# MeshFEM/MeshFEM

Measured on AMD Instinct MI355X. Metric: stiffness_assembly_elements_per_s, higher is better.
Workload: dtype f64; 1 GPU; configs[2]: 60^3 grid -> 5184000 P2 tets, isotropic E=200 nu=0.35, Dirichlet x=0, traction x=1; elements=5184000, nodes=7430761, dof=22292283, nnz_blocks=201443041, stored_blocks=104436901, matrix_storage=upper, parallelism=1 GPU, step=embed + Ke blocks + assembly into block-CSR (gather/owner-computes)

## Files before the change

### meshfem_amd/csrc/mfh_api.cpp

```cpp
#include "mfh_ctx.hh"
#include <dlfcn.h>

using namespace mfh;

namespace {
struct RoctxApi {
    int (*push)(const char *) = nullptr;
    int (*pop)() = nullptr;
    RoctxApi() {
        const char *en = getenv("MFH_ROCTX");
        if (!en || en[0] == '0') return;
        for (const char *lib : {"librocprofiler-sdk-roctx.so", "libroctx64.so", "/opt/rocm/lib/librocprofiler-sdk-roctx.so", "/opt/rocm/lib/libroctx64.so"}) {
            if (void *h = dlopen(lib, RTLD_NOW | RTLD_GLOBAL)) {
                push = reinterpret_cast<int (*)(const char *)>(dlsym(h, "roctxRangePushA"));
                pop = reinterpret_cast<int (*)()>(dlsym(h, "roctxRangePop"));
                if (push && pop) return;
                push = nullptr; pop = nullptr;
            }
        }
    }
};
RoctxApi &roctx_api() { static RoctxApi a; return a; }
}
mfh::RoctxRange::RoctxRange(const char *name) {
// ... 68 lines not shown
    double t0 = now_ms();
    c->autoStretch = -1.0;
    drop_p1_view(c);
    c->opDegree = 0;
    c->nodePairsValid = false;
    sampler_drop(c);
    if (!c->hostOnly && !deviceTables) {
        require_device(c);
        MFH_HIP(hipSetDevice(c->device));
        c->dElemNodes.upload(c->mesh.elemNodes, c->stream);
        c->dVertPos.upload(c->mesh.nodePos, c->stream);
    }
    c->timing.upload_ms = now_ms() - t0;
    c->haveMesh = true;
    c->external = false;
    c->geoValid = false;
    c->hGeoValid = false;
    c->dofForNode.clear();
    c->nDoF = c->mesh.nNode;
    build_shape_tables(c->mesh.dim, c->mesh.deg, c->tables);
    if (!c->hostOnly) { c->dPairTable.upload(c->tables.pairTable, c->stream); c->dMassTable.upload(c->tables.massRef, c->stream); }
    invalidate_symbolic(c);
    dist_detach(c);
    reset_bcs(c);
    clear_fixed(c);
}

void set_isotropic(mfh_ctx *c, double E, double nu) {
    double lam = (nu * E) / ((1.0 + nu) * (1.0 - 2.0 * nu));
    if (c->haveMesh && c->mesh.dim == 2) lam = (nu * E) / (1.0 - nu * nu);
    c->matMode = 0;
    c->matKind = MAT_ISO;
    c->matParams = {lam, E / (2.0 + 2.0 * nu), E, nu};
    c->geoValid = false;
    c->hGeoValid = false;
    invalidate_matrix(c);
}

void drop_p1_view(mfh_ctx *c) {
    if (c->p1) { mfh_destroy(c->p1); c->p1 = nullptr; }
    c->p1GeoGen = -1;
}

mfh_ctx *p1_view(mfh_ctx *c) {
    if (!c || c->opDegree != 1 || !c->p1) return nullptr;
    mfh_ctx *v = c->p1;
    if (!c->hostOnly) {
        ensure_geometry(c);
        v->dGeo.borrow(c->dGeo.p, c->dGeo.n);
        v->geoStride = c->geoStride;
        v->geoValid = true;
        if (v->dVertPos.borrowed || !v->dVertPos.p) v->dVertPos.borrow(c->dVertPos.p, (size_t)v->mesh.nNode * v->mesh.dim);
        if (c->p1GeoGen != c->geoGen) { invalidate_matrix(v); c->p1GeoGen = c->geoGen; }
    }
    return v;
}

void ensure_pass_events(mfh_ctx *c) {
    if (c->passEv[0]) return;
    for (auto &e : c->passEv) MFH_HIP(hipEventCreate(&e));
    MFH_HIP(hipHostMalloc((void **)&c->negHost, 2 * sizeof(int), hipHostMallocDefault));
}

void ensure_geometry(mfh_ctx *c, bool deferCheck) {
    require(c->haveMesh, MFH_ERR_STATE, "no mesh set");
    if (c->geoValid) return;
    require(!c->hostOnly, MFH_ERR_HIP, "host-only context (device -1): no HIP device, and there is no CPU fallback");
    require_device(c);
    MFH_HIP(hipSetDevice(c->device));
    const HostMesh &m = c->mesh;
    if (c->matParams.empty() && !c->dMatBorrowed) set_isotropic(c, 1.0, 0.3);
    if (c->matMode == 0 && !c->dMatBorrowed) {
        double E = c->matParams[2], nu = c->matParams[3];
        double lam = (nu * E) / ((1.0 + nu) * (1.0 - 2.0 * nu));
        if (m.dim == 2) lam = (nu * E) / (1.0 - nu * nu);
        c->matParams[0] = lam;
    }
    c->geoStride = c->matKind == MAT_ISO ? GEO_ISO_STRIDE : (c->matKind == MAT_ORTHO ? GEO_ORTHO_STRIDE : GEO_GEN_STRIDE);
    if (!c->dMatBorrowed) c->dMatParams.upload(c->matParams, c->stream);
    const double *dMat = c->dMatBorrowed ? c->dMatBorrowed : c->dMatParams.p;
    c->dGeo.alloc((size_t)m.nElem * c->geoStride);
    c->dNeg.alloc(2);
    c->dNeg.zero(c->stream);
    ensure_pass_events(c);
    MFH_HIP(hipEventRecord(c->passEv[0], c->stream));
    k::launch_geometry(m.dim, m.deg, c->matKind, m.nElem, c->dElemNodes.p, m.npe, c->dVertPos.p, dMat, c->matMode,
                       c->dGeo.p, c->geoStride, c->dNeg.p, c->stream);
    MFH_HIP(hipEventRecord(c->passEv[1], c->stream));
    MFH_HIP(hipMemcpyAsync(c->negHost, c->dNeg.p, 2 * sizeof(int), hipMemcpyDeviceToHost, c->stream));
    c->geoPending = true;
    if (!deferCheck) finish_geometry(c);
}

void finish_geometry(mfh_ctx *c) {
    if (!c->geoPending) return;
    c->geoPending = false;
    MFH_HIP(hipStreamSynchronize(c->stream));
    float ms = 0;
    MFH_HIP(hipEventElapsedTime(&ms, c->passEv[0], c->passEv[1]));
    c->timing.geometry_ms = ms;
    const int neg[2] = {c->negHost[0], c->negHost[1]};
    if (neg[0] > 0)
        throw Error(MFH_ERR_INVALID, "Mesh has negatively oriented elements.\nCorrect with: mesh_convert --reorientNegativeElements. (" +
                                         std::to_string(neg[0]) + " elements)");
    if (neg[1] > 0)
        throw Error(MFH_ERR_INVALID, std::string(c->matMode == 1 ? "Isotropic" : "Orthotropic") + " parameters of " + std::to_string(neg[1]) +
                                         " elements give an indefinite elasticity tensor (" +
                                         (c->matMode == 1 ? "need E > 0 and -1 < nu < 1/2, nu < 1 in plane stress" : "compliance matrix not positive definite") + ").");
    c->geoValid = true;
    c->hGeoValid = false;
    ++c->geoGen;
}

const std::vector<double> &host_geo(mfh_ctx *c) {
    ensure_geometry(c);
    if (!c->hGeoValid) {
        c->hGeo.resize(c->dGeo.n);
        c->dGeo.download(c->hGeo.data(), c->dGeo.n, c->stream);
        c->hGeoValid = true;
    }
    return c->hGeo;
}

const int32_t *device_dof_map(mfh_ctx *c) {
    if (c->dofForNode.empty()) return nullptr;
    if (!c->dofUploaded) { c->dDofForNode.upload(c->dofForNode, c->stream); c->dofUploaded = true; }
    return c->dDofForNode.p;
}

void ensure_host_colidx(mfh_ctx *c) {
    if (!c->sym.colIdx.empty() || c->sym.nnzb == 0) return;
    c->sym.colIdx.resize((size_t)c->sym.nnzb);
    c->dColIdx.download(c->sym.colIdx.data(), c->sym.colIdx.size(), c->stream);
}
// ... 78 lines not shown
    flag.alloc(1);
    c->codesPacked = k::launch_pack_codes(c->sym.nChunk(), c->dContribPtr.p, c->dContribCode.p, c->mesh.npe, c->dChunkElemBase.p, flag.p, c->stream);
}

void ensure_node_pairs(mfh_ctx *c) {
    if (c->nodePairsValid) return;
    const HostMesh &m = c->mesh;
    const int npe = m.npe;
    std::vector<int32_t> ptr((size_t)m.nNode + 1, 0), pairs((size_t)m.nElem * npe);
    require((int64_t)pairs.size() <= 2147483647LL, MFH_ERR_UNSUPPORTED, "more than 2^31 (element, node) pairs");
    for (size_t k2 = 0; k2 < pairs.size(); ++k2) ++ptr[(size_t)m.elemNodes[k2] + 1];
    for (int64_t n = 0; n < m.nNode; ++n) ptr[(size_t)n + 1] += ptr[(size_t)n];
    std::vector<int32_t> cur(ptr.begin(), ptr.end() - 1);
    for (size_t k2 = 0; k2 < pairs.size(); ++k2) pairs[(size_t)cur[(size_t)m.elemNodes[k2]]++] = (int32_t)k2;
    c->dNodePtr.upload(ptr, c->stream);
    c->dNodePair.upload(pairs, c->stream);
    c->nodePairsValid = true;
}

k::AsmArgs asm_args(mfh_ctx *c) {
    const HostMesh &m = c->mesh;
    k::AsmArgs a{};
    a.dim = m.dim; a.deg = m.deg; a.npe = m.npe; a.mat = c->asmMat();
    a.geoStride = c->geoStride; a.geo = c->dGeo.p; a.pairTable = c->dPairTable.p; a.massTable = c->dMassTable.p;
    for (int k2 = 0; k2 < 6; ++k2) a.pairConst[k2] = c->tables.pairConst[k2];
    a.nChunk = c->sym.nChunk(); a.chunkRow = c->dChunkRow.p; a.rowPtr = c->dRowPtr.p;
    a.contribPtr = c->dContribPtr.p; a.contribCode = c->dContribCode.p; a.contribSlot = c->dContribSlot.p;
    a.chunkSlots = c->sym.chunkSlots;
    a.nElem = m.nElem; a.scatterSlot = c->dScatter.p;
    a.vals = c->dVals.p; a.nnzb = c->sym.nnzb;
    a.xcd = c->xcdSwizzle;
    a.upperOnly = c->upperOnly ? 1 : 0;
    a.det = c->deterministic ? 1 : 0;
    a.chunkElemBase = c->codesPacked ? c->dChunkElemBase.p : nullptr;
    a.chunkOrder = nullptr;
    if (c->asmChunkOrder && !c->hostOnly && a.nChunk > 1 && c->symValid && c->dContribPtr.p && c->dContribCode.p && c->contribOrder == 1) {
        if (c->chunkOrderGen != c->listsGen) {
            DBuf<uint32_t> keys;
            keys.alloc((size_t)a.nChunk);
            k::launch_chunk_keys(a, keys.p, c->stream);
            std::vector<uint32_t> hk((size_t)a.nChunk);
            keys.download(hk.data(), hk.size(), c->stream);
            std::vector<int32_t> order((size_t)a.nChunk);
            for (int64_t b = 0; b < a.nChunk; ++b) order[(size_t)b] = (int32_t)b;
            std::stable_sort(order.begin(), order.end(), [&](int32_t x, int32_t y) { return hk[(size_t)x] < hk[(size_t)y]; });
            c->dChunkOrder.upload(order, c->stream);
            c->chunkOrderGen = c->listsGen;
        }
        a.chunkOrder = c->dChunkOrder.p;
    }
    return a;
}

void run_assembly(mfh_ctx *c, int mode) {
    c->dVals32.release();
    k::AsmArgs a = asm_args(c);
    if (mode == MFH_ASSEMBLE_ATOMIC) {
        c->dVals.zero(c->stream);
        k::launch_assemble_atomic(a, c->stream);
    } else {
        k::launch_assemble_gather(a, c->stream);
    }
}

void placement_trials(mfh_ctx *c) {
    c->placementGen = c->valsGen;
// ... 866 lines not shown
    MFH_TRY(c)
    require(c && out, MFH_ERR_INVALID, "null argument");
    const std::vector<double> &g = host_geo(c);
    for (int64_t e = 0; e < c->mesh.nElem; ++e) out[e] = g[(size_t)e * c->geoStride + 12];
    MFH_CATCH(c)
}

mfh_status mfh_material_isotropic(mfh_ctx *c, double E, double nu) {
    MFH_TRY(c)
    require(c, MFH_ERR_INVALID, "null context");
    set_isotropic(c, E, nu);
    MFH_CATCH(c)
}

mfh_status mfh_material_const(mfh_ctx *c, const double *D) {
    MFH_TRY(c)
    require(c && D && c->haveMesh, MFH_ERR_STATE, "set the mesh before the material");
    const int d = c->dim(), fl = flat_len(d);
    c->matParams.clear();
    bool ortho = true;
    for (int r = 0; r < fl && ortho; ++r)
        for (int cc = r + 1; cc < fl; ++cc)
            if (cc >= d && D[r * fl + cc] != 0.0) { ortho = false; break; }
    if (ortho) {
        for (int r = 0; r < d; ++r)
            for (int cc = r; cc < d; ++cc) c->matParams.push_back(D[r * fl + cc]);
        for (int k2 = d; k2 < fl; ++k2) c->matParams.push_back(D[k2 * fl + k2]);
        c->matMode = 5; c->matKind = MAT_ORTHO;
    } else {
        for (int r = 0; r < fl; ++r)
            for (int cc = r; cc < fl; ++cc) c->matParams.push_back(D[r * fl + cc]);
        c->matMode = 2; c->matKind = MAT_GENERAL;
    }
    c->geoValid = false; c->hGeoValid = false;
    invalidate_matrix(c);
    MFH_CATCH(c)
}

mfh_status mfh_material_iso_field(mfh_ctx *c, const double *E, const double *nu) {
    MFH_TRY(c)
    require(c && E && nu && c->haveMesh, MFH_ERR_STATE, "set the mesh before the material");
    const int64_t n = c->mesh.nElem;
    c->matParams.assign((size_t)2 * n, 0.0);
    std::copy(E, E + n, c->matParams.begin());
    std::copy(nu, nu + n, c->matParams.begin() + n);
    c->matMode = 1; c->matKind = MAT_ISO;
    c->geoValid = false; c->hGeoValid = false;
    invalidate_matrix(c);
    MFH_CATCH(c)
}

mfh_status mfh_material_ortho_field(mfh_ctx *c, const double *params) {
    MFH_TRY(c)
    require(c && params && c->haveMesh, MFH_ERR_STATE, "set the mesh before the material");
    const int np = c->dim() == 3 ? 9 : 4;
    c->matParams.assign(params, params + (size_t)np * c->mesh.nElem);
    c->matMode = 3; c->matKind = MAT_ORTHO;
    c->geoValid = false; c->hGeoValid = false;
    invalidate_matrix(c);
    MFH_CATCH(c)
}

mfh_status mfh_material_tensor_field(mfh_ctx *c, const double *D) {
    MFH_TRY(c)
    require(c && D && c->haveMesh, MFH_ERR_STATE, "set the mesh before the material");
    const int fl = flat_len(c->dim());
    c->matParams.assign(D, D + (size_t)fl * fl * c->mesh.nElem);
    c->matMode = 4; c->matKind = MAT_GENERAL;
    c->geoValid = false; c->hGeoValid = false;
    invalidate_matrix(c);
    MFH_CATCH(c)
}

mfh_status mfh_material_get(mfh_ctx *c, int64_t elem, double *D) {
    MFH_TRY(c)
    require(c && D && c->haveMesh && elem >= 0 && elem < c->mesh.nElem, MFH_ERR_INVALID, "bad element");
    const std::vector<double> &g = host_geo(c);
    elem_D(c, &g[(size_t)elem * c->geoStride], D);
    MFH_CATCH(c)
}

mfh_status mfh_dof_map(mfh_ctx *c, const int32_t *dofForNode, int64_t nDoF) {
    MFH_TRY(c)
    require(!(c && c->opDegree == 1 && c->p1), MFH_ERR_STATE, "a forced-degree-1 view is in force (mfh_set_operator_degree): it is defined for the identity DoF map");
    require(c && c->haveMesh, MFH_ERR_STATE, "no mesh set");
    c->nOwnedDoFSet = -1;
    if (!dofForNode) {
        c->dofForNode.clear();
        c->nDoF = c->mesh.nNode;
        std::fill(c->mesh.bdryInternal.begin(), c->mesh.bdryInternal.end(), (uint8_t)0);
    } else {
        require(c->mesh.nOwned == c->mesh.nNode, MFH_ERR_UNSUPPORTED, "a DoF map on a partitioned mesh says which DoFs are this rank's rows: mfh_dof_map_partitioned");
        require(nDoF > 0 && nDoF <= c->mesh.nNode, MFH_ERR_INVALID, "bad nDoF");
        for (int64_t n = 0; n < c->mesh.nNode; ++n)
            require(dofForNode[n] >= 0 && dofForNode[n] < nDoF, MFH_ERR_INVALID, "DoF index out of range");
        c->dofForNode.assign(dofForNode, dofForNode + c->mesh.nNode);
        c->nDoF = nDoF;
    }
    invalidate_symbolic(c);
    clear_fixed(c);
    MFH_CATCH(c)
}
// ... 921 lines not shown
```

### meshfem_amd/csrc/mfh_ctx.hh

```
#pragma once
#include "mfh_internal.hh"
#include <cmath>
#include <map>
#include <mutex>

using namespace mfh;

struct mfh_ctx {
    int device = 0;
    bool hostOnly = false;
    bool hierarchyLevel = false;
    bool keepHostSymbolic = false;
    int xcdSwizzle = 0;
    RawVec<double> hLoad, hX, hXBatch, hLoadBatch;
    bool alwaysReembed = false;
    bool deterministic = false;
    DBuf<double> detPartials;
    DBuf<unsigned> detCounter;
    bool periodicIgnoreMismatch = false;
    int periodicIgnoreDims = 0;
    hipStream_t stream = nullptr;
    bool ownStream = true;
    bool arenaCounted = false;
    std::string err;

    HostMesh mesh;
    bool haveMesh = false;
    bool external = false;
    DBuf<int32_t> dElemNodes;
    DBuf<double> dVertPos;

    int matMode = 0;
    int matKind = MAT_ISO;
    int op = MFH_OP_ELASTICITY;
    int opDegree = 0;
    mfh_ctx *p1 = nullptr;
    int64_t geoGen = 0, p1GeoGen = -1;
    DBuf<int32_t> dNodePtr, dNodePair;
    bool nodePairsValid = false;
    struct SamplerGrid {
        bool valid = false;
        int nc[3] = {1, 1, 1};
        double org[3] = {0, 0, 0}, hi[3] = {0, 0, 0}, cs[3] = {1, 1, 1};
        int64_t nItems = 0, nPairs = 0, maxPop = 0;
        double buildMs = 0, hostMs = 0;
        DBuf<int32_t> cellStart, items;
        void reset() { valid = false; nItems = nPairs = maxPop = 0; buildMs = hostMs = 0; cellStart.release(); items.release(); }
    };
    struct Sampler {
        SamplerGrid elem, bdry;
        double pad = 0;
        double bbMin[3] = {0, 0, 0}, bbMax[3] = {0, 0, 0};
        DBuf<int32_t> bdryVerts, bdryParent;
    } sampler;
    double samplerCellScale = 1.0;
    std::vector<double> matParams;
    DBuf<double> dMatParams;
    const double *dMatBorrowed = nullptr;
    DBuf<double> dGeo;
    DBuf<int> dNeg;
    int geoStride = GEO_ISO_STRIDE;
    bool geoValid = false;
    hipEvent_t passEv[4] = {nullptr, nullptr, nullptr, nullptr};
    int *negHost = nullptr;
    bool geoPending = false;
    std::vector<double> hGeo;
    bool hGeoValid = false;

    std::vector<int32_t> dofForNode;
    DBuf<int32_t> dDofForNode;
    bool dofUploaded = false;
    int64_t nDoF = 0;

    Symbolic sym;
    bool symValid = false;
    bool symHasScatter = false;
    DBuf<int32_t> dRowPtr, dColIdx, dChunkRow, dSpmvChunkRow, dScatter;
    DBuf<int64_t> dContribPtr;
    int matrixStorage = -1;
    bool upperOnly = false;
    int nCU = 256;
    DBuf<uint32_t> dContribCode;
    DBuf<uint16_t> dContribSlot;
    ShapeTables tables;
    DBuf<double> dPairTable, dMassTable;
    MfLists mf;
    bool mfValid = false;
    int matrixFree = -1;
    bool use_mf() const {
        if (external || !haveMesh || hostOnly || kron()) return false;
        return matrixFree == 1 || (matrixFree < 0 && op == MFH_OP_ELASTICITY);
    }
    DBuf<int32_t> dMfChunkRow;
// ... 328 lines not shown
```

### meshfem_amd/csrc/mfh_internal.hh

```
#pragma once
#include <hip/hip_runtime.h>
#include <cstdint>
#include <cstdio>
#include <cstring>
#include <string>
#include <vector>
#include <stdexcept>
#include <chrono>
#include <thread>
#include <functional>
#include <algorithm>
#include <array>
#include <memory>
#include <cstdlib>
#include "../../include/meshfem_hip.h"
#include "../../include/meshfem_hip_extras.h"

namespace mfh {

struct Error : std::runtime_error {
    mfh_status code;
    Error(mfh_status c, const std::string &m) : std::runtime_error(m), code(c) {}
};

// ... 293 lines not shown
struct DetScope {
    DetBuf saved;
    explicit DetScope(const DetBuf &d) : saved(t_det) { t_det = d; }
    ~DetScope() { t_det = saved; }
    DetScope(const DetScope &) = delete;
    DetScope &operator=(const DetScope &) = delete;
};
inline int det_grid(int grid) { return t_det.partials ? std::min(grid, t_det.cap) : grid; }
void launch_det_finish(hipStream_t s);

struct AsmArgs {
    int dim, deg, npe, mat;
    int geoStride;
    const double *geo;
    const double *pairTable;
    const double *massTable;
    double pairConst[6];
    int64_t nChunk;
    const int32_t *chunkRow;
    const int32_t *rowPtr;
    const int64_t *contribPtr;
    const uint32_t *contribCode;
    const uint16_t *contribSlot;
    int chunkSlots;
    int64_t nElem;
    const int32_t *scatterSlot;
    double *vals;
    int64_t nnzb;
    int xcd;
    const int32_t *chunkElemBase;
    const int32_t *chunkOrder;
    int upperOnly;
    int det;
};

void launch_geometry(int dim, int deg, int mat, int64_t nElem, const int32_t *elemNodes, int npe,
                     const double *vertPos, const double *matParams, int matMode, double *geo, int geoStride,
                     int *negCount, hipStream_t s);
void launch_assemble_gather(const AsmArgs &a, hipStream_t s);
void launch_chunk_keys(const AsmArgs &a, uint32_t *keys, hipStream_t s);
bool launch_pack_codes(int64_t nChunk, const int64_t *contribPtr, uint32_t *contribCode, int npe, int32_t *chunkElemBase, int *flag, hipStream_t s);
void launch_assemble_atomic(const AsmArgs &a, hipStream_t s);
void launch_element_stiffness(const AsmArgs &a, int64_t first, int64_t count, double *KeOut, hipStream_t s);
void launch_constant_strain_load(const AsmArgs &a, const int32_t *elemNodes, const int32_t *dofForNode, const double *intGrad,
                                 const double *cstrain, const double *deltaP, double *out, hipStream_t s);
void launch_average_strain(const AsmArgs &a, const int32_t *elemNodes, const double *intGrad, const double *uNodes, double *out,
                           int wantStress, const double *uFixed, const double *deltaP, hipStream_t s, const double *addStrain = nullptr,
                           double *integral = nullptr);
void launch_apply_delta_K(const AsmArgs &a, const int32_t *elemNodes, const int32_t *dofForNode, const double *intGrad,
                          const double *uNodes, const double *deltaP, double *out, hipStream_t s);
void launch_mutual_energies(const AsmArgs &a, const int32_t *elemNodes, const double *intGrad, const double *w, int64_t nNode,
                            const double *deltaP, double *out, hipStream_t s);
void launch_boundary_strain_field(const AsmArgs &a, const int32_t *elemNodes, const double *intGrad, int64_t nBE,
                                  const int32_t *bdryParent, const int32_t *bdryElemNodes, int npbe, const double *uNodes,
                                  int wantStress, double *out, hipStream_t s);
void launch_strain_field(const AsmArgs &a, const int32_t *elemNodes, const double *intGrad, const double *uNodes, int wantStress,
                         double *out, hipStream_t s);
void launch_sym_measures(int dim, int64_t n, const double *field, int what, double *vm, double *eval, double *evec, hipStream_t s);
void launch_stress_measures(const AsmArgs &a, const int32_t *elemNodes, const double *intGrad, const double *uNodes, int wantStress, int what,
                            double *vm, double *eval, double *evec, hipStream_t s);
constexpr int PEAK_GRID_CAP = 1024;
void launch_peak_von_mises(const AsmArgs &a, const int32_t *elemNodes, const double *intGrad, const double *uNodes, int wantStress,
                           double *partV, int64_t *partI, double *outV, int64_t *outI, hipStream_t s);
void launch_vertex_average(int dim, int npe, int64_t nVert, const int32_t *nodePtr, const int32_t *nodePair, const double *geo, int geoStride,
                           const double *field, int nq, int nComp, double *out, hipStream_t s);
void launch_mutual_energy_differential(const AsmArgs &a, const int32_t *elemNodes, const double *intGrad, const double *w,
// ... 186 lines not shown
```

### meshfem_amd/csrc/mfh_kernels.hip

```cpp
#include "mfh_device.hh"

namespace mfh { namespace k {

template <int DIM, int MAT> DEV constexpr int mat_nb() { return (MAT == MAT_LAPLACE || MAT == MAT_MASS) ? 1 : DIM * DIM; }

template <int DIM, int MAT>
DEV void block_from_H(const double *__restrict__ g, const double (&H)[DIM][DIM], double *K);

template <int DIM>
DEV void pair_H(const double *__restrict__ g, uint32_t offs , double S0, double S1, double S2,
                double S3, double (&H)[DIM][DIM]) {
#ifndef MFH_ASM_ABLATE
#define MFH_ASM_ABLATE 0
#endif
    const double vol = MFH_ASM_ABLATE >= 1 ? 1.0 : g[12];
    S0 *= vol; S1 *= vol; S2 *= vol; S3 *= vol;
    const char *gb = reinterpret_cast<const char *>(g);
    const double *gsi = reinterpret_cast<const double *>(gb + (offs & 0xffu)), *gti = reinterpret_cast<const double *>(gb + ((offs >> 8) & 0xffu)),
                 *gsj = reinterpret_cast<const double *>(gb + ((offs >> 16) & 0xffu)), *gtj = reinterpret_cast<const double *>(gb + (offs >> 24));
    double ua[DIM], ub[DIM], p[DIM], q[DIM];
#pragma unroll
    for (int a = 0; a < DIM; ++a) {
        ua[a] = MFH_ASM_ABLATE >= 1 ? S0 + a : gsi[a]; ub[a] = MFH_ASM_ABLATE >= 1 ? S1 - a : gti[a];
        const double va = MFH_ASM_ABLATE >= 2 ? S2 + a : gsj[a], vb = MFH_ASM_ABLATE >= 2 ? S3 - a : gtj[a];
        p[a] = S0 * va + S1 * vb;
        q[a] = S2 * va + S3 * vb;
    }
#pragma unroll
    for (int a = 0; a < DIM; ++a)
#pragma unroll
        for (int b = 0; b < DIM; ++b) H[a][b] = ua[a] * p[b] + ub[a] * q[b];
}

template <int DIM, int DEG, int MAT>
DEV void elem_block(const double *__restrict__ g, const double *__restrict__ pairTab, const PairConst &pc, int i, int j, double *K) {
    constexpr int NPE = (DIM == 3) ? (DEG == 1 ? 4 : 10) : (DEG == 1 ? 3 : 6);
    const double vol = g[12];
    if (MAT == MAT_MASS) {
        K[0] = vol * pairTab[i * NPE + j];
        return;
    }
    double H[DIM][DIM];
    if (DEG == 1) {
        double gi[DIM], gj[DIM];
#pragma unroll
        for (int a = 0; a < DIM; ++a) { gi[a] = g[i * DIM + a]; gj[a] = g[j * DIM + a] * vol; }
#pragma unroll
        for (int a = 0; a < DIM; ++a)
#pragma unroll
            for (int b = 0; b < DIM; ++b) H[a][b] = gi[a] * gj[b];
    } else {
        const int si = sup_s<DIM, DEG>(i), ti = sup_t<DIM, DEG>(i), sj = sup_s<DIM, DEG>(j), tj = sup_t<DIM, DEG>(j);
        constexpr int NV = DIM + 1;
        const bool vi = i < NV, vj = j < NV;
        const int lAi = vi ? si : ti, lBi = si, lAj = vj ? sj : tj, lBj = sj;
        const double c1 = pc.ee_ne, c2 = pc.ee_eq - pc.ee_ne, c3 = pc.ee_ne - pc.ve_ne;
        const double oi = vi ? 1.0 : 0.0, oj = vj ? 1.0 : 0.0;
        auto coef = [&](bool eq, double o, double o2) -> double { return (c1 + (eq ? c2 : 0.0)) - c3 * (o + o2) + o * o2; };
        double S0 = coef(lAi == lAj, oi, oj);
        double S1 = vj ? 0.0 : coef(lAi == lBj, oi, 0.0);
        double S2 = vi ? 0.0 : coef(lBi == lAj, 0.0, oj);
        double S3 = (vi | vj) ? 0.0 : coef(lBi == lBj, 0.0, 0.0);
        S0 *= vol; S1 *= vol; S2 *= vol; S3 *= vol;
        double ua[DIM], ub[DIM], p[DIM], q[DIM];
#pragma unroll
        for (int a = 0; a < DIM; ++a) {
            ua[a] = g[si * DIM + a]; ub[a] = g[ti * DIM + a];
            const double va = g[sj * DIM + a], vb = g[tj * DIM + a];
            p[a] = S0 * va + S1 * vb;
            q[a] = S2 * va + S3 * vb;
        }
#pragma unroll
        for (int a = 0; a < DIM; ++a)
#pragma unroll
            for (int b = 0; b < DIM; ++b) H[a][b] = ua[a] * p[b] + ub[a] * q[b];
    }
    block_from_H<DIM, MAT>(g, H, K);
}

template <int DIM, int MAT>
DEV void block_from_H(const double *__restrict__ g, const double (&H)[DIM][DIM], double *K) {
    if (MAT == MAT_LAPLACE) {
        double tr = 0;
#pragma unroll
        for (int a = 0; a < DIM; ++a) tr += H[a][a];
        K[0] = tr;
    } else if (MAT == MAT_ISO) {
#if defined(MFH_ASM_ABLATE) && MFH_ASM_ABLATE >= 1
        const double lam = H[0][0], mu = H[1][1];
#else
        const double lam = g[13], mu = g[14];
#endif
        double tr = 0;
#pragma unroll
        for (int a = 0; a < DIM; ++a) tr += H[a][a];
#pragma unroll
        for (int c = 0; c < DIM; ++c)
#pragma unroll
            for (int d = 0; d < DIM; ++d) K[c * DIM + d] = lam * H[c][d] + mu * H[d][c] + (c == d ? mu * tr : 0.0);
    } else if (MAT == MAT_ORTHO) {
#pragma unroll
        for (int c = 0; c < DIM; ++c)
#pragma unroll
            for (int d = 0; d < DIM; ++d) {
                double v = g[13 + npack<DIM>(c, d)] * H[c][d];
                if (c == d) {
#pragma unroll
                    for (int a = 0; a < DIM; ++a)
                        if (a != c) v += g[ortho_shear_offset<DIM>() + flat_idx<DIM>(a, c) - DIM] * H[a][a];
                } else v += g[ortho_shear_offset<DIM>() + flat_idx<DIM>(c, d) - DIM] * H[d][c];
                K[c * DIM + d] = v;
            }
    } else {
        constexpr int ND = (DIM * (DIM + 1) / 2) * (DIM * (DIM + 1) / 2 + 1) / 2;
        double D[ND];
#pragma unroll
        for (int k = 0; k < ND; ++k) D[k] = g[13 + k];
#pragma unroll
        for (int c = 0; c < DIM; ++c)
#pragma unroll
            for (int d = 0; d < DIM; ++d) {
                double acc = 0;
#pragma unroll
                for (int a = 0; a < DIM; ++a)
#pragma unroll
                    for (int b = 0; b < DIM; ++b) acc += H[a][b] * D[dpack<DIM>(flat_idx<DIM>(a, c), flat_idx<DIM>(d, b))];
                K[c * DIM + d] = acc;
            }
    }
}

template <int DIM>
DEV void embed_simplex(const double (&P)[DIM + 1][DIM], double (&gl)[DIM + 1][DIM], double &vol) {
    if (DIM == 3) {
        auto cross = [](const double *a, const double *b, double *o) {
            o[0] = a[1] * b[2] - a[2] * b[1]; o[1] = a[2] * b[0] - a[0] * b[2]; o[2] = a[0] * b[1] - a[1] * b[0];
        };
        double d31[3], d21[3], d01[3], d20[3], d30[3], d10[3], n[4][3];
#pragma unroll
        for (int a = 0; a < 3; ++a) {
            d31[a] = P[3][a] - P[1][a]; d21[a] = P[2][a] - P[1][a]; d01[a] = P[0][a] - P[1][a];
            d20[a] = P[2][a] - P[0][a]; d30[a] = P[3][a] - P[0][a]; d10[a] = P[1][a] - P[0][a];
        }
        cross(d31, d21, n[0]); cross(d20, d30, n[1]); cross(d30, d10, n[2]); cross(d10, d20, n[3]);
        const double vol6 = d01[0] * n[0][0] + d01[1] * n[0][1] + d01[2] * n[0][2];
        vol = vol6 / 6.0;
#pragma unroll
        for (int k = 0; k < 4; ++k)
#pragma unroll
            for (int a = 0; a < 3; ++a) gl[k][a] = n[k][a] / vol6;
    } else {
        double E[3][2];
#pragma unroll
        for (int a = 0; a < 2; ++a) { E[0][a] = P[2][a] - P[1][a]; E[1][a] = P[0][a] - P[2][a]; E[2][a] = P[1][a] - P[0][a]; }
        const double dA = E[1][0] * E[2][1] - E[1][1] * E[2][0];
        vol = dA / 2.0;
#pragma unroll
        for (int k = 0; k < 3; ++k) { gl[k][0] = -E[k][1] / dA; gl[k][1] = E[k][0] / dA; }
    }
}

template <int DIM>
// ... 46 lines not shown
            const double c11 = a00 * a22 - a02 * a02, c12 = a01 * a02 - a00 * a12, c22 = a00 * a11 - a01 * a01;
            const double det = a00 * c00 + a01 * c01 + a02 * c02;
            if (!(a00 > 0 && c22 > 0 && det > 0 && q[6] > 0 && q[7] > 0 && q[8] > 0)) atomicAdd(negCount + 1, 1);
            g[13 + npack<3>(0, 0)] = c00 / det; g[13 + npack<3>(0, 1)] = c01 / det; g[13 + npack<3>(0, 2)] = c02 / det;
            g[13 + npack<3>(1, 1)] = c11 / det; g[13 + npack<3>(1, 2)] = c12 / det; g[13 + npack<3>(2, 2)] = c22 / det;
            g[ortho_shear_offset<3>() + 0] = q[6]; g[ortho_shear_offset<3>() + 1] = q[7]; g[ortho_shear_offset<3>() + 2] = q[8];
        } else {
            const double *q = mp + e * 4;
            const double a00 = 1.0 / q[0], a01 = -q[2] / q[1], a11 = 1.0 / q[1];
            const double det = a00 * a11 - a01 * a01;
            if (!(a00 > 0 && det > 0 && q[3] > 0)) atomicAdd(negCount + 1, 1);
            g[13 + npack<2>(0, 0)] = a11 / det; g[13 + npack<2>(0, 1)] = -a01 / det; g[13 + npack<2>(1, 1)] = a00 / det;
            g[ortho_shear_offset<2>()] = q[3];
        }
    } else {
        const double *q = mp + e * FL * FL;
        for (int r = 0; r < FL; ++r)
            for (int c = r; c < FL; ++c) g[13 + dpack<DIM>(r, c)] = q[r * FL + c];
    }
    }
    __syncthreads();
    const int64_t e0 = (int64_t)blockIdx.x * blockDim.x;
    const int nLive = (int)(nElem - e0 < (int64_t)blockDim.x ? nElem - e0 : (int64_t)blockDim.x);
    double *out = geo + e0 * stride;
    for (int q = threadIdx.x; q < nLive * stride; q += blockDim.x) {
        const int el = q / stride;
        out[q] = recs[(size_t)el * (stride + 1) + (q - el * stride)];
    }
}

template <int DIM, int DEG, int MAT> DEV constexpr bool asm_uses_table() { return DEG == 2 && MAT != MAT_MASS; }
constexpr int ASM_CODE_SHIFT = 7;

template <int DIM, int DEG, int MAT, bool UPPER = false, bool DET = false>
__global__ void __launch_bounds__(256, (MAT == MAT_GENERAL || MAT == MAT_ORTHO) ? 1 : 8) k_assemble_gather(AsmArgs a) {
    constexpr int NB = mat_nb<DIM, MAT>();
    constexpr int NPE = (DIM == 3) ? (DEG == 1 ? 4 : 10) : (DEG == 1 ? 3 : 6);
    constexpr bool TAB = asm_uses_table<DIM, DEG, MAT>();
    extern __shared__ __attribute__((aligned(16))) double acc[];
    const int CS = a.chunkSlots + 2;
    double *tabS = acc + (size_t)NB * CS;
    uint32_t *tabO = reinterpret_cast<uint32_t *>(tabS + NPE * NPE * 4);
    uint32_t *turn = tabO + NPE * NPE;
    const PairConst pc{a.pairConst[0], a.pairConst[1], a.pairConst[2], a.pairConst[3], a.pairConst[4], a.pairConst[5]};
    const int64_t item = a.xcd == 1 ? xcd_item(blockIdx.x, gridDim.x) : (a.xcd > 1 ? xcd_group_item(blockIdx.x, gridDim.x, a.xcd) : (int64_t)blockIdx.x);
    const int64_t chunk = a.chunkOrder ? (int64_t)a.chunkOrder[item] : item;
    const int r0 = a.chunkRow[chunk], r1 = a.chunkRow[chunk + 1];
    const int s0 = a.rowPtr[r0];
    const int ns = a.rowPtr[r1] - s0;
    const uint32_t eBase = a.chunkElemBase ? (uint32_t)a.chunkElemBase[chunk] : 0u;
    const int par = s0 & 1;
    for (int t = threadIdx.x; t < ns + par; t += 256)
#pragma unroll
        for (int c = 0; c < NB; ++c) acc[c * CS + t] = 0.0;
    if (DET && threadIdx.x == 0) *turn = 0u;
    if (TAB) {
        for (int t = threadIdx.x; t < NPE * NPE; t += 256) {
            const int i = t / NPE, j = t - i * NPE;
#pragma unroll
            for (int k = 0; k < 4; ++k) tabS[t * 4 + k] = a.pairTable[t * 4 + k];
            tabO[t] = (uint32_t)(sup_s<DIM, DEG>(i) * DIM * 8) | ((uint32_t)(sup_t<DIM, DEG>(i) * DIM * 8) << 8) |
                      ((uint32_t)(sup_s<DIM, DEG>(j) * DIM * 8) << 16) | ((uint32_t)(sup_t<DIM, DEG>(j) * DIM * 8) << 24);
        }
    }
    __syncthreads();
    const int64_t kb = a.contribPtr[chunk], ke = a.contribPtr[chunk + 1];
    constexpr int U = 2;
    constexpr bool det = DET;
    unsigned turnNo = threadIdx.x >> 6;
    for (int64_t k0 = kb + threadIdx.x; det ? (k0 - threadIdx.x < ke) : (k0 < ke); k0 += 256 * U) {
        uint32_t code[U];
        int ls[U];
        bool ok[U];
#pragma unroll
        for (int u = 0; u < U; ++u) {
            const int64_t kk = k0 + (int64_t)u * 256;
            ok[u] = kk < ke;
            code[u] = ok[u] ? a.contribCode[kk] : a.contribCode[kb];
            ls[u] = (ok[u] ? (int)a.contribSlot[kk] : 0) + par;
        }
#pragma unroll
        for (int u = 0; u < U; ++u) {
            double K[NB];
            if (ok[u]) {
            uint32_t e;
            int ij;
            if (a.chunkElemBase) { e = eBase + (code[u] >> ASM_CODE_SHIFT); ij = (int)(code[u] & ((1u << ASM_CODE_SHIFT) - 1)); }
            else { e = code[u] / (NPE * NPE); ij = (int)(code[u] - e * (NPE * NPE)); }
            const double *g = a.geo + (int64_t)e * a.geoStride;
            if (TAB) {
                typedef double dv2 __attribute__((ext_vector_type(2)));
                const dv2 s01 = *reinterpret_cast<const dv2 *>(&tabS[ij * 4]), s23 = *reinterpret_cast<const dv2 *>(&tabS[ij * 4 + 2]);
                const uint32_t offs = tabO[ij];
                double H[DIM][DIM];
                pair_H<DIM>(g, offs, s01.x, s01.y, s23.x, s23.y, H);
                block_from_H<DIM, MAT>(g, H, K);
            } else {
                const int i = ij / NPE, j = ij - i * NPE;
                elem_block<DIM, DEG, MAT>(g, MAT == MAT_MASS ? a.massTable : a.pairTable, pc, i, j, K);
            }
            }
            if (det) {
                if ((threadIdx.x & 63) == 0)
                    while (__hip_atomic_load(turn, __ATOMIC_ACQUIRE, __HIP_MEMORY_SCOPE_WORKGROUP) != turnNo) __builtin_amdgcn_s_sleep(1);
                if (ok[u]) {
#pragma unroll
                    for (int c = 0; c < NB; ++c) unsafeAtomicAdd(&acc[c * CS + ls[u]], K[c]);
                }
                __builtin_amdgcn_fence(__ATOMIC_RELEASE, "workgroup");
                if ((threadIdx.x & 63) == 0) __hip_atomic_store(turn, turnNo + 1u, __ATOMIC_RELEASE, __HIP_MEMORY_SCOPE_WORKGROUP);
                turnNo += 4u;
            } else if (ok[u]) {
#pragma unroll
                for (int c = 0; c < NB; ++c) unsafeAtomicAdd(&acc[c * CS + ls[u]], K[c]);
            }
            __builtin_amdgcn_sched_barrier(0);
        }
    }
    __syncthreads();
    const int nl = ns + par;
    const int64_t sbase = (int64_t)s0 - par;
    const int pfirst = par;
    const int plast = nl >> 1;
    for (int p = pfirst + threadIdx.x; p < plast; p += 256) {
        const int t = 2 * p;
        const int64_t s = sbase + t;
#pragma unroll
        for (int c = 0; c < NB; ++c) {
            const double2 v = *reinterpret_cast<const double2 *>(&acc[c * CS + t]);
            double2 *dst = reinterpret_cast<double2 *>(&a.vals[tiled_index(s, c, NB)]);
            typedef double dv2 __attribute__((ext_vector_type(2)));
            dv2 w = {v.x, v.y};
            __builtin_nontemporal_store(w, reinterpret_cast<dv2 *>(dst));
        }
    }
    if (threadIdx.x < 2) {
        const int t = threadIdx.x == 0 ? 1 : nl - 1;
        const bool live = threadIdx.x == 0 ? (par == 1 && nl > 1) : ((nl & 1) && nl - 1 >= par && !(par == 1 && nl - 1 == 1));
        if (live) {
            const int64_t s = sbase + t;
#pragma unroll
            for (int c = 0; c < NB; ++c) a.vals[tiled_index(s, c, NB)] = acc[c * CS + t];
        }
    }
}

__global__ void __launch_bounds__(256) k_chunk_keys(int64_t nChunk, const int64_t *__restrict__ contribPtr, const uint32_t *__restrict__ contribCode,
                                                    const int32_t *__restrict__ chunkElemBase, uint32_t npe2, uint32_t *__restrict__ keys) {
    const int64_t b = (int64_t)blockIdx.x * 256 + threadIdx.x;
    if (b >= nChunk) return;
    const int64_t kb = contribPtr[b], ke = contribPtr[b + 1];
    if (ke <= kb) { keys[b] = 0xffffffffu; return; }
    const uint32_t c = contribCode[kb + (ke - kb) / 2];
    keys[b] = chunkElemBase ? (uint32_t)chunkElemBase[b] + (c >> ASM_CODE_SHIFT) : c / npe2;
}

__global__ void __launch_bounds__(64) k_pack_codes(int64_t nChunk, const int64_t *__restrict__ contribPtr, uint32_t *__restrict__ contribCode,
                                                   uint32_t npe2, int32_t *__restrict__ chunkElemBase, int *flag, int rewrite) {
    const int64_t b = blockIdx.x;
    const int64_t kb = contribPtr[b], ke = contribPtr[b + 1];
    if (rewrite) {
        const uint32_t lo = (uint32_t)chunkElemBase[b];
        for (int64_t k = kb + threadIdx.x; k < ke; k += 64) {
            const uint32_t c = contribCode[k], e = c / npe2;
            contribCode[k] = ((e - lo) << ASM_CODE_SHIFT) | (c - e * npe2);
        }
        return;
    }
    uint32_t lo = 0xffffffffu, hi = 0;
    for (int64_t k = kb + threadIdx.x; k < ke; k += 64) {
        const uint32_t e = contribCode[k] / npe2;
        lo = e < lo ? e : lo;
        hi = e > hi ? e : hi;
    }
#pragma unroll
    for (int off = 32; off > 0; off >>= 1) {
        const uint32_t l2 = __shfl_xor(lo, off, 64), h2 = __shfl_xor(hi, off, 64);
// ... 1887 lines not shown
        case 3: { CALL(3, 2, MAT_ISO); } break;                                           \
        case 4: { CALL(3, 2, MAT_GENERAL); } break;                                       \
        case 5: { CALL(3, 2, MAT_ORTHO); } break;                                         \
        case 6: { CALL(2, 1, MAT_ISO); } break;                                           \
        case 7: { CALL(2, 1, MAT_GENERAL); } break;                                       \
        case 8: { CALL(2, 1, MAT_ORTHO); } break;                                         \
        case 9: { CALL(2, 2, MAT_ISO); } break;                                           \
        case 10: { CALL(2, 2, MAT_GENERAL); } break;                                      \
        default: { CALL(2, 2, MAT_ORTHO); } break;                                        \
        }                                                                                \
    } while (0)

#define MFH_DISPATCH_ASM(a, CALL)                                                        \
    do {                                                                                 \
        if (!mat_is_scalar(a.mat)) { MFH_DISPATCH(a, CALL); break; }                     \
        const int key_ = (a.dim == 3 ? 0 : 4) + (a.deg == 2 ? 2 : 0) + (a.mat == MAT_MASS ? 1 : 0); \
        switch (key_) {                                                                  \
        case 0: { CALL(3, 1, MAT_LAPLACE); } break;                                       \
        case 1: { CALL(3, 1, MAT_MASS); } break;                                          \
        case 2: { CALL(3, 2, MAT_LAPLACE); } break;                                       \
        case 3: { CALL(3, 2, MAT_MASS); } break;                                          \
        case 4: { CALL(2, 1, MAT_LAPLACE); } break;                                       \
        case 5: { CALL(2, 1, MAT_MASS); } break;                                          \
        case 6: { CALL(2, 2, MAT_LAPLACE); } break;                                       \
        default: { CALL(2, 2, MAT_MASS); } break;                                         \
        }                                                                                \
    } while (0)

void launch_assemble_gather(const AsmArgs &a, hipStream_t s) {
    if (a.nChunk == 0) return;
    size_t lds = (size_t)(mat_is_scalar(a.mat) ? 1 : a.dim * a.dim) * (a.chunkSlots + 2) * sizeof(double);
    if (a.deg == 2 && a.mat != MAT_MASS) lds += (size_t)a.npe * a.npe * (4 * sizeof(double) + sizeof(uint32_t));
    if (a.det) lds = (size_t)(mat_is_scalar(a.mat) ? 1 : a.dim * a.dim) * (a.chunkSlots + 2) * sizeof(double) + (size_t)a.npe * a.npe * (4 * sizeof(double) + sizeof(uint32_t)) + 16;
#define CALLV(D, G, M, UP, DT)                                                                                 \
    do {                                                                                                         \
        if (lds > 64 * 1024)                                                                                     \
            MFH_HIP(hipFuncSetAttribute((const void *)k_assemble_gather<D, G, M, UP, DT>, hipFuncAttributeMaxDynamicSharedMemorySize, (int)lds)); \
        hipLaunchKernelGGL((k_assemble_gather<D, G, M, UP, DT>), dim3((unsigned)a.nChunk), dim3(256), lds, s, a); \
    } while (0)
#define CALL(D, G, M)                                                     \
    if (a.det) { if (a.upperOnly) CALLV(D, G, M, true, true); else CALLV(D, G, M, false, true); } \
    else { if (a.upperOnly) CALLV(D, G, M, true, false); else CALLV(D, G, M, false, false); }
    MFH_DISPATCH_ASM(a, CALL);
#undef CALL
#undef CALLV
    CHECK_LAUNCH();
}

void launch_chunk_keys(const AsmArgs &a, uint32_t *keys, hipStream_t s) {
    if (a.nChunk == 0) return;
    hipLaunchKernelGGL(k_chunk_keys, dim3((unsigned)((a.nChunk + 255) / 256)), dim3(256), 0, s, a.nChunk, a.contribPtr, a.contribCode,
                       a.chunkElemBase, (uint32_t)(a.npe * a.npe), keys);
    CHECK_LAUNCH();
}

bool launch_pack_codes(int64_t nChunk, const int64_t *contribPtr, uint32_t *contribCode, int npe, int32_t *chunkElemBase, int *flag, hipStream_t s) {
    if (nChunk == 0) return true;
    MFH_HIP(hipMemsetAsync(flag, 0, sizeof(int), s));
    hipLaunchKernelGGL(k_pack_codes, dim3((unsigned)nChunk), dim3(64), 0, s, nChunk, contribPtr, contribCode, (uint32_t)(npe * npe), chunkElemBase, flag, 0);
    CHECK_LAUNCH();
    int h = 0;
    MFH_HIP(hipMemcpyAsync(&h, flag, sizeof(int), hipMemcpyDeviceToHost, s));
    MFH_HIP(hipStreamSynchronize(s));
    if (h) return false;
    hipLaunchKernelGGL(k_pack_codes, dim3((unsigned)nChunk), dim3(64), 0, s, nChunk, contribPtr, contribCode, (uint32_t)(npe * npe), chunkElemBase, flag, 1);
    CHECK_LAUNCH();
    return true;
}

void launch_assemble_atomic(const AsmArgs &a, hipStream_t s) {
    const int64_t total = a.nElem * a.npe * a.npe;
    const int grid = grid_for(total, 256 * 32);
#define CALL(D, G, M) hipLaunchKernelGGL((k_assemble_atomic<D, G, M>), dim3(grid), dim3(256), 0, s, a)
    MFH_DISPATCH_ASM(a, CALL);
#undef CALL
    CHECK_LAUNCH();
}
// ... 435 lines not shown
```

Baseline: 1.551 billion elements/s.

## Apply constant material tensor once per assembled block instead of per element contribution

When the elasticity material is uniform (isotropic/general constant), the gather assembly kernel now accumulates the raw geometric H matrices across element contributions and applies the material tensor map once per output block at write-out. Material constants are passed by value in the kernel arguments. This removes the per-contribution lambda/mu multiply work and per-element material reads. It also avoids re-uploading material params and re-zeroing the negative-element counter on repeated geometry builds. The negative-element check now tracks deltas across calls, which adds bookkeeping and risk.

```diff
diff --git a/meshfem_amd/csrc/mfh_api.cpp b/meshfem_amd/csrc/mfh_api.cpp
--- a/meshfem_amd/csrc/mfh_api.cpp
+++ b/meshfem_amd/csrc/mfh_api.cpp
@@ -124,6 +124,7 @@
     c->matMode = 0;
     c->matKind = MAT_ISO;
     c->matParams = {lam, E / (2.0 + 2.0 * nu), E, nu};
+    c->matUploaded = false;
     c->geoValid = false;
     c->hGeoValid = false;
     invalidate_matrix(c);
@@ -166,14 +167,18 @@
         double E = c->matParams[2], nu = c->matParams[3];
         double lam = (nu * E) / ((1.0 + nu) * (1.0 - 2.0 * nu));
         if (m.dim == 2) lam = (nu * E) / (1.0 - nu * nu);
+        if (c->matParams[0] != lam) c->matUploaded = false;
         c->matParams[0] = lam;
     }
     c->geoStride = c->matKind == MAT_ISO ? GEO_ISO_STRIDE : (c->matKind == MAT_ORTHO ? GEO_ORTHO_STRIDE : GEO_GEN_STRIDE);
-    if (!c->dMatBorrowed) c->dMatParams.upload(c->matParams, c->stream);
+    if (!c->dMatBorrowed && !(c->matUploaded && c->dMatParams.p)) { c->dMatParams.upload(c->matParams, c->stream); c->matUploaded = true; }
     const double *dMat = c->dMatBorrowed ? c->dMatBorrowed : c->dMatParams.p;
     c->dGeo.alloc((size_t)m.nElem * c->geoStride);
-    c->dNeg.alloc(2);
-    c->dNeg.zero(c->stream);
+    if (!c->dNeg.p || c->geoPending) {
+        c->dNeg.alloc(2);
+        c->dNeg.zero(c->stream);
+        c->negSeen[0] = c->negSeen[1] = 0u;
+    }
     ensure_pass_events(c);
     MFH_HIP(hipEventRecord(c->passEv[0], c->stream));
     k::launch_geometry(m.dim, m.deg, c->matKind, m.nElem, c->dElemNodes.p, m.npe, c->dVertPos.p, dMat, c->matMode,
@@ -191,7 +196,11 @@
     float ms = 0;
     MFH_HIP(hipEventElapsedTime(&ms, c->passEv[0], c->passEv[1]));
     c->timing.geometry_ms = ms;
-    const int neg[2] = {c->negHost[0], c->negHost[1]};
+    int neg[2];
+    for (int k2 = 0; k2 < 2; ++k2) {
+        neg[k2] = (int)((unsigned)c->negHost[k2] - c->negSeen[k2]);
+        c->negSeen[k2] = (unsigned)c->negHost[k2];
+    }
     if (neg[0] > 0)
         throw Error(MFH_ERR_INVALID, "Mesh has negatively oriented elements.\nCorrect with: mesh_convert --reorientNegativeElements. (" +
                                          std::to_string(neg[0]) + " elements)");
@@ -336,6 +345,12 @@
     a.xcd = c->xcdSwizzle;
     a.upperOnly = c->upperOnly ? 1 : 0;
     a.det = c->deterministic ? 1 : 0;
+    if (c->op == MFH_OP_ELASTICITY && (c->geoValid || c->geoPending) && !c->dMatBorrowed && (c->matMode == 0 || c->matMode == 2 || c->matMode == 5)) {
+        const size_t np = c->matMode == 0 ? 2 : c->matParams.size();
+        require(np <= sizeof(a.matConst) / sizeof(double) && np <= c->matParams.size(), MFH_ERR_STATE, "constant material: unexpected parameter count");
+        a.constMat = 1;
+        std::copy(c->matParams.begin(), c->matParams.begin() + (ptrdiff_t)np, a.matConst);
+    }
     a.chunkElemBase = c->codesPacked ? c->dChunkElemBase.p : nullptr;
     a.chunkOrder = nullptr;
     if (c->asmChunkOrder && !c->hostOnly && a.nChunk > 1 && c->symValid && c->dContribPtr.p && c->dContribCode.p && c->contribOrder == 1) {
@@ -1268,7 +1283,7 @@
             for (int cc = r; cc < fl; ++cc) c->matParams.push_back(D[r * fl + cc]);
         c->matMode = 2; c->matKind = MAT_GENERAL;
     }
-    c->geoValid = false; c->hGeoValid = false;
+    c->geoValid = false; c->hGeoValid = false; c->matUploaded = false;
     invalidate_matrix(c);
     MFH_CATCH(c)
 }
@@ -1281,7 +1296,7 @@
     std::copy(E, E + n, c->matParams.begin());
     std::copy(nu, nu + n, c->matParams.begin() + n);
     c->matMode = 1; c->matKind = MAT_ISO;
-    c->geoValid = false; c->hGeoValid = false;
+    c->geoValid = false; c->hGeoValid = false; c->matUploaded = false;
     invalidate_matrix(c);
     MFH_CATCH(c)
 }
@@ -1292,7 +1307,7 @@
     const int np = c->dim() == 3 ? 9 : 4;
     c->matParams.assign(params, params + (size_t)np * c->mesh.nElem);
     c->matMode = 3; c->matKind = MAT_ORTHO;
-    c->geoValid = false; c->hGeoValid = false;
+    c->geoValid = false; c->hGeoValid = false; c->matUploaded = false;
     invalidate_matrix(c);
     MFH_CATCH(c)
 }
@@ -1303,7 +1318,7 @@
     const int fl = flat_len(c->dim());
     c->matParams.assign(D, D + (size_t)fl * fl * c->mesh.nElem);
     c->matMode = 4; c->matKind = MAT_GENERAL;
-    c->geoValid = false; c->hGeoValid = false;
+    c->geoValid = false; c->hGeoValid = false; c->matUploaded = false;
     invalidate_matrix(c);
     MFH_CATCH(c)
 }
diff --git a/meshfem_amd/csrc/mfh_ctx.hh b/meshfem_amd/csrc/mfh_ctx.hh
--- a/meshfem_amd/csrc/mfh_ctx.hh
+++ b/meshfem_amd/csrc/mfh_ctx.hh
@@ -56,9 +56,11 @@
     double samplerCellScale = 1.0;
     std::vector<double> matParams;
     DBuf<double> dMatParams;
+    bool matUploaded = false;
     const double *dMatBorrowed = nullptr;
     DBuf<double> dGeo;
     DBuf<int> dNeg;
+    unsigned negSeen[2] = {0u, 0u};
     int geoStride = GEO_ISO_STRIDE;
     bool geoValid = false;
     hipEvent_t passEv[4] = {nullptr, nullptr, nullptr, nullptr};
diff --git a/meshfem_amd/csrc/mfh_internal.hh b/meshfem_amd/csrc/mfh_internal.hh
--- a/meshfem_amd/csrc/mfh_internal.hh
+++ b/meshfem_amd/csrc/mfh_internal.hh
@@ -349,6 +349,8 @@
     const int32_t *chunkOrder;
     int upperOnly;
     int det;
+    int constMat;
+    double matConst[21];
 };
 
 void launch_geometry(int dim, int deg, int mat, int64_t nElem, const int32_t *elemNodes, int npe,
diff --git a/meshfem_amd/csrc/mfh_kernels.hip b/meshfem_amd/csrc/mfh_kernels.hip
--- a/meshfem_amd/csrc/mfh_kernels.hip
+++ b/meshfem_amd/csrc/mfh_kernels.hip
@@ -4,6 +4,8 @@
 
 template <int DIM, int MAT> DEV constexpr int mat_nb() { return (MAT == MAT_LAPLACE || MAT == MAT_MASS) ? 1 : DIM * DIM; }
 
+template <int DIM, int MAT>
+DEV void tensor_map(const double *__restrict__ mp, const double (&H)[DIM][DIM], double *K);
 template <int DIM, int MAT>
 DEV void block_from_H(const double *__restrict__ g, const double (&H)[DIM][DIM], double *K);
 
@@ -32,15 +34,9 @@
         for (int b = 0; b < DIM; ++b) H[a][b] = ua[a] * p[b] + ub[a] * q[b];
 }
 
-template <int DIM, int DEG, int MAT>
-DEV void elem_block(const double *__restrict__ g, const double *__restrict__ pairTab, const PairConst &pc, int i, int j, double *K) {
-    constexpr int NPE = (DIM == 3) ? (DEG == 1 ? 4 : 10) : (DEG == 1 ? 3 : 6);
+template <int DIM, int DEG>
+DEV void elem_H(const double *__restrict__ g, const PairConst &pc, int i, int j, double (&H)[DIM][DIM]) {
     const double vol = g[12];
-    if (MAT == MAT_MASS) {
-        K[0] = vol * pairTab[i * NPE + j];
-        return;
-    }
-    double H[DIM][DIM];
     if (DEG == 1) {
         double gi[DIM], gj[DIM];
 #pragma unroll
@@ -75,6 +71,17 @@
 #pragma unroll
             for (int b = 0; b < DIM; ++b) H[a][b] = ua[a] * p[b] + ub[a] * q[b];
     }
+}
+
+template <int DIM, int DEG, int MAT>
+DEV void elem_block(const double *__restrict__ g, const double *__restrict__ pairTab, const PairConst &pc, int i, int j, double *K) {
+    constexpr int NPE = (DIM == 3) ? (DEG == 1 ? 4 : 10) : (DEG == 1 ? 3 : 6);
+    if (MAT == MAT_MASS) {
+        K[0] = g[12] * pairTab[i * NPE + j];
+        return;
+    }
+    double H[DIM][DIM];
+    elem_H<DIM, DEG>(g, pc, i, j, H);
     block_from_H<DIM, MAT>(g, H, K);
 }
 
@@ -85,49 +92,45 @@
 #pragma unroll
         for (int a = 0; a < DIM; ++a) tr += H[a][a];
         K[0] = tr;
-    } else if (MAT == MAT_ISO) {
+    } else tensor_map<DIM, MAT>(g + 13, H, K);
+}
+
+template <int DIM, int MAT>
+DEV double tensor_map_entry(const double *__restrict__ mp, const double (&H)[DIM][DIM], int c, int d) {
+    if (MAT == MAT_ISO) {
 #if defined(MFH_ASM_ABLATE) && MFH_ASM_ABLATE >= 1
         const double lam = H[0][0], mu = H[1][1];
 #else
-        const double lam = g[13], mu = g[14];
+        const double lam = mp[0], mu = mp[1];
 #endif
         double tr = 0;
 #pragma unroll
         for (int a = 0; a < DIM; ++a) tr += H[a][a];
-#pragma unroll
-        for (int c = 0; c < DIM; ++c)
-#pragma unroll
-            for (int d = 0; d < DIM; ++d) K[c * DIM + d] = lam * H[c][d] + mu * H[d][c] + (c == d ? mu * tr : 0.0);
+        return lam * H[c][d] + mu * H[d][c] + (c == d ? mu * tr : 0.0);
     } else if (MAT == MAT_ORTHO) {
-#pragma unroll
-        for (int c = 0; c < DIM; ++c)
-#pragma unroll
-            for (int d = 0; d < DIM; ++d) {
-                double v = g[13 + npack<DIM>(c, d)] * H[c][d];
-                if (c == d) {
-#pragma unroll
-                    for (int a = 0; a < DIM; ++a)
-                        if (a != c) v += g[ortho_shear_offset<DIM>() + flat_idx<DIM>(a, c) - DIM] * H[a][a];
-                } else v += g[ortho_shear_offset<DIM>() + flat_idx<DIM>(c, d) - DIM] * H[d][c];
-                K[c * DIM + d] = v;
-            }
+        double v = mp[npack<DIM>(c, d)] * H[c][d];
+        if (c == d) {
+#pragma unroll
+            for (int a = 0; a < DIM; ++a)
+                if (a != c) v += mp[ortho_shear_offset<DIM>() - 13 + flat_idx<DIM>(a, c) - DIM] * H[a][a];
+        } else v += mp[ortho_shear_offset<DIM>() - 13 + flat_idx<DIM>(c, d) - DIM] * H[d][c];
+        return v;
     } else {
-        constexpr int ND = (DIM * (DIM + 1) / 2) * (DIM * (DIM + 1) / 2 + 1) / 2;
-        double D[ND];
-#pragma unroll
-        for (int k = 0; k < ND; ++k) D[k] = g[13 + k];
-#pragma unroll
-        for (int c = 0; c < DIM; ++c)
-#pragma unroll
-            for (int d = 0; d < DIM; ++d) {
-                double acc = 0;
-#pragma unroll
-                for (int a = 0; a < DIM; ++a)
-#pragma unroll
-                    for (int b = 0; b < DIM; ++b) acc += H[a][b] * D[dpack<DIM>(flat_idx<DIM>(a, c), flat_idx<DIM>(d, b))];
-                K[c * DIM + d] = acc;
-            }
-    }
+        double acc = 0;
+#pragma unroll
+        for (int a = 0; a < DIM; ++a)
+#pragma unroll
+            for (int b = 0; b < DIM; ++b) acc += H[a][b] * mp[dpack<DIM>(flat_idx<DIM>(a, c), flat_idx<DIM>(d, b))];
+        return acc;
+    }
+}
+
+template <int DIM, int MAT>
+DEV void tensor_map(const double *__restrict__ mp, const double (&H)[DIM][DIM], double *K) {
+#pragma unroll
+    for (int c = 0; c < DIM; ++c)
+#pragma unroll
+        for (int d = 0; d < DIM; ++d) K[c * DIM + d] = tensor_map_entry<DIM, MAT>(mp, H, c, d);
 }
 
 template <int DIM>
@@ -240,8 +243,8 @@
 template <int DIM, int DEG, int MAT> DEV constexpr bool asm_uses_table() { return DEG == 2 && MAT != MAT_MASS; }
 constexpr int ASM_CODE_SHIFT = 7;
 
-template <int DIM, int DEG, int MAT, bool UPPER = false, bool DET = false>
-__global__ void __launch_bounds__(256, (MAT == MAT_GENERAL || MAT == MAT_ORTHO) ? 1 : 8) k_assemble_gather(AsmArgs a) {
+template <int DIM, int DEG, int MAT, bool UPPER, bool DET, bool CONSTMAT>
+DEV void assemble_gather(const AsmArgs &a) {
     constexpr int NB = mat_nb<DIM, MAT>();
     constexpr int NPE = (DIM == 3) ? (DEG == 1 ? 4 : 10) : (DEG == 1 ? 3 : 6);
     constexpr bool TAB = asm_uses_table<DIM, DEG, MAT>();
@@ -302,10 +305,18 @@
                 const uint32_t offs = tabO[ij];
                 double H[DIM][DIM];
                 pair_H<DIM>(g, offs, s01.x, s01.y, s23.x, s23.y, H);
-                block_from_H<DIM, MAT>(g, H, K);
+                if constexpr (CONSTMAT) {
+#pragma unroll
+                    for (int c = 0; c < NB; ++c) K[c] = H[c / DIM][c % DIM];
+                } else block_from_H<DIM, MAT>(g, H, K);
             } else {
                 const int i = ij / NPE, j = ij - i * NPE;
-                elem_block<DIM, DEG, MAT>(g, MAT == MAT_MASS ? a.massTable : a.pairTable, pc, i, j, K);
+                if constexpr (CONSTMAT) {
+                    double H[DIM][DIM];
+                    elem_H<DIM, DEG>(g, pc, i, j, H);
+#pragma unroll
+                    for (int c = 0; c < NB; ++c) K[c] = H[c / DIM][c % DIM];
+                } else elem_block<DIM, DEG, MAT>(g, MAT == MAT_MASS ? a.massTable : a.pairTable, pc, i, j, K);
             }
             }
             if (det) {
@@ -333,13 +344,28 @@
     for (int p = pfirst + threadIdx.x; p < plast; p += 256) {
         const int t = 2 * p;
         const int64_t s = sbase + t;
+        typedef double dv2 __attribute__((ext_vector_type(2)));
+        if constexpr (CONSTMAT) {
+            double H0[DIM][DIM], H1[DIM][DIM];
+#pragma unroll
+            for (int c = 0; c < NB; ++c) {
+                const double2 v = *reinterpret_cast<const double2 *>(&acc[c * CS + t]);
+                H0[c / DIM][c % DIM] = v.x; H1[c / DIM][c % DIM] = v.y;
+            }
+#pragma unroll
+            for (int c = 0; c < NB; ++c) {
+                dv2 w = {tensor_map_entry<DIM, MAT>(a.matConst, H0, c / DIM, c % DIM), tensor_map_entry<DIM, MAT>(a.matConst, H1, c / DIM, c % DIM)};
+                __builtin_nontemporal_store(w, reinterpret_cast<dv2 *>(&a.vals[tiled_index(s, c, NB)]));
+                __builtin_amdgcn_sched_barrier(0);
+            }
+        } else {
 #pragma unroll
         for (int c = 0; c < NB; ++c) {
             const double2 v = *reinterpret_cast<const double2 *>(&acc[c * CS + t]);
             double2 *dst = reinterpret_cast<double2 *>(&a.vals[tiled_index(s, c, NB)]);
-            typedef double dv2 __attribute__((ext_vector_type(2)));
             dv2 w = {v.x, v.y};
             __builtin_nontemporal_store(w, reinterpret_cast<dv2 *>(dst));
+        }
         }
     }
     if (threadIdx.x < 2) {
@@ -347,10 +373,28 @@
         const bool live = threadIdx.x == 0 ? (par == 1 && nl > 1) : ((nl & 1) && nl - 1 >= par && !(par == 1 && nl - 1 == 1));
         if (live) {
             const int64_t s = sbase + t;
+            if constexpr (CONSTMAT) {
+                double H[DIM][DIM], K[NB];
+#pragma unroll
+                for (int c = 0; c < NB; ++c) H[c / DIM][c % DIM] = acc[c * CS + t];
+                tensor_map<DIM, MAT>(a.matConst, H, K);
+#pragma unroll
+                for (int c = 0; c < NB; ++c) a.vals[tiled_index(s, c, NB)] = K[c];
+            } else {
 #pragma unroll
             for (int c = 0; c < NB; ++c) a.vals[tiled_index(s, c, NB)] = acc[c * CS + t];
-        }
-    }
+            }
+        }
+    }
+}
+
+template <int DIM, int DEG, int MAT, bool UPPER = false, bool DET = false>
+__global__ void __launch_bounds__(256, (MAT == MAT_GENERAL || MAT == MAT_ORTHO) ? 1 : 8) k_assemble_gather(AsmArgs a) {
+    assemble_gather<DIM, DEG, MAT, UPPER, DET, false>(a);
+}
+template <int DIM, int DEG, int MAT, bool UPPER = false, bool DET = false>
+__global__ void __launch_bounds__(256, 8) k_assemble_gather_const(AsmArgs a) {
+    assemble_gather<DIM, DEG, MAT, UPPER, DET, true>(a);
 }
 
 __global__ void __launch_bounds__(256) k_chunk_keys(int64_t nChunk, const int64_t *__restrict__ contribPtr, const uint32_t *__restrict__ contribCode,
@@ -2304,17 +2348,25 @@
     size_t lds = (size_t)(mat_is_scalar(a.mat) ? 1 : a.dim * a.dim) * (a.chunkSlots + 2) * sizeof(double);
     if (a.deg == 2 && a.mat != MAT_MASS) lds += (size_t)a.npe * a.npe * (4 * sizeof(double) + sizeof(uint32_t));
     if (a.det) lds = (size_t)(mat_is_scalar(a.mat) ? 1 : a.dim * a.dim) * (a.chunkSlots + 2) * sizeof(double) + (size_t)a.npe * a.npe * (4 * sizeof(double) + sizeof(uint32_t)) + 16;
-#define CALLV(D, G, M, UP, DT)                                                                                 \
+#define CALLV(KERN, D, G, M, UP, DT)                                                                           \
     do {                                                                                                         \
         if (lds > 64 * 1024)                                                                                     \
-            MFH_HIP(hipFuncSetAttribute((const void *)k_assemble_gather<D, G, M, UP, DT>, hipFuncAttributeMaxDynamicSharedMemorySize, (int)lds)); \
-        hipLaunchKernelGGL((k_assemble_gather<D, G, M, UP, DT>), dim3((unsigned)a.nChunk), dim3(256), lds, s, a); \
+            MFH_HIP(hipFuncSetAttribute((const void *)KERN<D, G, M, UP, DT>, hipFuncAttributeMaxDynamicSharedMemorySize, (int)lds)); \
+        hipLaunchKernelGGL((KERN<D, G, M, UP, DT>), dim3((unsigned)a.nChunk), dim3(256), lds, s, a);           \
     } while (0)
-#define CALL(D, G, M)                                                     \
-    if (a.det) { if (a.upperOnly) CALLV(D, G, M, true, true); else CALLV(D, G, M, false, true); } \
-    else { if (a.upperOnly) CALLV(D, G, M, true, false); else CALLV(D, G, M, false, false); }
-    MFH_DISPATCH_ASM(a, CALL);
+#define CALLK(KERN, D, G, M)                                              \
+    if (a.det) { if (a.upperOnly) CALLV(KERN, D, G, M, true, true); else CALLV(KERN, D, G, M, false, true); } \
+    else { if (a.upperOnly) CALLV(KERN, D, G, M, true, false); else CALLV(KERN, D, G, M, false, false); }
+    if (a.constMat && !mat_is_scalar(a.mat)) {
+#define CALL(D, G, M) CALLK(k_assemble_gather_const, D, G, M)
+        MFH_DISPATCH(a, CALL);
 #undef CALL
+    } else {
+#define CALL(D, G, M) CALLK(k_assemble_gather, D, G, M)
+        MFH_DISPATCH_ASM(a, CALL);
+#undef CALL
+    }
+#undef CALLK
 #undef CALLV
     CHECK_LAUNCH();
 }
```

Result: faster. 1.634 billion elements/s (median of 6 runs) (+5.4%).
